# Qervas/cn_chess_ai

Hardware: AMD Instinct MI355X
Metric: env steps/sec + DQN updates/sec at 8192 parallel games, 1/2/4/8 MI355X (higher is better)
Workload: dtype f32

## Files before the change

### cn_chess_ai_amd/csrc/xq_dqn.hip

```cpp
#include "xq_internal.h"
#include <hip/hip_ext.h>
#include "xq_gemm.hip.h"
#include "xq_screen.hip.h"
#include "xq_gemm_dma.hip.h"
#include "xq_l0grad.hip.h"

#include <algorithm>
#include <cmath>
#include <mutex>
#include <random>
#include <unordered_map>

namespace xq { struct TailArgs; struct ClipRecord; }
struct xq_dqn {
    int ns = 0, nl = 0;
    int L[XQ_MAX_LAYERS + 1] = {0};
    size_t nw = 0, nb = 0;
    size_t wo[XQ_MAX_LAYERS] = {0}, bo[XQ_MAX_LAYERS] = {0};
    double lr = 1e-3, gamma = 0.99;
    uint64_t seed = 0;
    hipStream_t stream = nullptr;
    bool own_stream = false;
    hipStream_t side = nullptr;
    hipStream_t cur = nullptr;
// ... 1452 lines not shown
        g.M = d->L[ll + 1]; g.N = d->L[ll]; g.K = n;
        g.A = d->deltas[ll]; g.lda = d->L[ll + 1];
        g.B = outs[ll - 1]; g.ldb = d->L[ll];
        return grad_gemm<L_MCONTIG>(d, g, G + d->g_wh[ll], "gemm_grad_hidden", d->slabs + off_h[ll], &d->pend_hidden[ll]);
    };
    const bool defer_grad = nl == 3;
    int waiting = -1;
    for (int l = nl - 3; l >= 0; --l) {
        tail_begin(d);
        XQ_TRY(hidden_deltas(d, n, d->deltas[l + 1], d->L[l + 2], d->L[l + 2], mode, l, l));
        if (defer_grad) { if (waiting >= 0) XQ_TRY(add_grad(waiting)); waiting = l + 1; }
        else XQ_TRY(add_grad(l + 1));
        if (l == nl - 3) add_out_grad();
        if (l == 0 && l0_mfma_shape(d, n)) {
            XQ_TRY(ensure_l0_mfma(d, n));
            TailArgs& T = *d->tail;
            const int chunk0 = l0_chunk_of(n), kpad = (n + chunk0 - 1) / chunk0 * chunk0;
            T.sel_boards = d->gboards; T.sel_n = n; T.sel_kpad = kpad; T.sel_out = d->l0_sel; T.n_sel = kpad / 64;
            d->tail_bytes += (double)n * 48 + 2.0 * l0sel_elems(kpad);
            d->tail_lds = std::max(d->tail_lds, (size_t)64 * 13 * sizeof(uint32_t));
            d->l0_sel_done = true;
        }
        XQ_TRY(tail_launch(d, false, "td_tail_deltas"));
    }
    tail_begin(d);
    XQ_TRY(l0_gradient(d, n, G + d->g_w0));
    if (waiting >= 0) XQ_TRY(add_grad(waiting));
    if (nl < 3) add_out_grad();
    BiasJobs bj;
    for (int l = 0; l <= nl - 2; ++l) bj.add(d->deltas[l], d->L[l + 1], d->L[l + 1], G + d->g_bh[l]);
    d->pend_bh = xq_dqn::PendingSlab();
    XQ_TRY(bias_grads(d, bj, n, &d->pend_bh));
    return tail_launch(d, true, "td_tail_l0");
}


struct TdStep {
    const int32_t* action_to; const float* reward; const uint8_t* done; SlotSrc slots; const PerOpts* per;
    int n, mode, sel_net, nl, Hl, NO; bool dbl, bf;
    bool big_tiles;
    int n_partial;
    size_t bias_lds;
    float* outs[XQ_MAX_LAYERS]; uint16_t* outs_bf[XQ_MAX_LAYERS];
    float* touts[XQ_MAX_LAYERS]; uint16_t* touts_bf[XQ_MAX_LAYERS];
    float* t2outs[XQ_MAX_LAYERS]; uint16_t* t2outs_bf[XQ_MAX_LAYERS];
    const float* view; long long view_ld; int view_kmax;
};

static int screen_guard_tick(xq_dqn* d, int n, bool* screened) {
    XQ_TRY(ensure_screen_capacity(d, n));
    if (d->scr_guard_pending && d->scr_host_steps % kScreenCheckEvery == 0 && d->scr_host_steps != d->scr_guard_queued_at) {
        XQ_HIP(hipEventSynchronize(d->scr_guard_ev));
        d->scr_guard_pending = false;
        unsigned long long h[2];
        screen_stat_sums_of(d, d->scr_guard_host, h);
        const double ds = (double)(d->scr_guard_samples - d->scr_seen[0]);
        if (ds > 0 && ((double)(h[0] - d->scr_seen[1]) > kScreenMaxPairs * ds || (double)(h[1] - d->scr_seen[2]) > kScreenMaxWhole * ds)) {
            d->scr_hold = kScreenHoldSteps;
            d->scr_fallbacks += 1;
        }
        if (ds > 0) {
            const double share = (double)(h[1] - d->scr_seen[2]) / ds;
            if (share > 0.25) d->scr_stage_whole = true; else if (share < 0.10) d->scr_stage_whole = false;
        }
        d->scr_seen[0] = d->scr_guard_samples; d->scr_seen[1] = h[0]; d->scr_seen[2] = h[1];
    }
    *screened = d->scr_hold == 0;
    if (d->scr_hold > 0) --d->scr_hold;
    return XQ_OK;
}

static int screen_shadow_job(xq_dqn* d, int sel_net, int parity, ShadowJob* shadow) {
    const int NO = d->nout(), nl = d->nl;
    const bool full = d->scr_static_net != sel_net;
    if (full) XQ_HIP(hipMemsetAsync(d->scr_wmax + 4, 0, 2 * sizeof(unsigned), d->cur));
    memset(shadow, 0, sizeof *shadow);
    shadow->W = d->wl(sel_net, nl - 1); shadow->bias = d->bl(sel_net, nl - 1); shadow->NO = NO; shadow->K = d->hlast(); shadow->Wb = d->scr_wb;
    shadow->w_dyn = d->scr_wmax + parity; shadow->b_dyn = d->scr_wmax + 2 + parity;
    shadow->w_stat = d->scr_wmax + 4; shadow->b_stat = d->scr_wmax + 5;
    shadow->nblocks = full ? (NO + kShadowRows - 1) / kShadowRows : std::min((int)kShadowDynBlocks, (NO + kShadowRows - 1) / kShadowRows);
    d->scr_static_net = sel_net;
    return XQ_OK;
}

static int launch_screen(xq_dqn* d, const ScreenArgs& a, int mode, hipEvent_t start, hipEvent_t stop) {
    using ScreenKernel = void (*)(ScreenArgs);
    static const ScreenKernel kerns[3][2] = {{screen_top2_kernel<1, 2, SCR_TOP2>, screen_top2_kernel<2, 1, SCR_TOP2>},
                                             {screen_top2_kernel<1, 2, SCR_ARG>, screen_top2_kernel<2, 1, SCR_ARG>},
                                             {screen_top2_kernel<1, 2, SCR_MAX>, screen_top2_kernel<2, 1, SCR_MAX>}};
    const ScreenKernel kern = kerns[mode][a.K == 256 ? 0 : 1];
    XQ_TRY(ensure_max_dynamic_lds(kern, 160 * 1024));
    hipExtLaunchKernelGGL(kern, dim3(a.panels * a.ranges), dim3(512), screen_lds_bytes(a), d->cur, start, stop, 0, a);
    XQ_HIP(hipGetLastError());
    return XQ_OK;
}

static int colmax_persistent_grid(const xq_dqn* d, GemmArgs& g, int tiles_m, int total) {
    g.a_vec = g.b_vec = 1; g.k_chunk = g.K;
    g.bias_padded = ((((uintptr_t)g.bias) % 16 == 0) && (g.M % 4) == 0) ? 1 : 0;
    const int grid = std::min(total, 2 * d->ncu);
    if (grid >= 2 && (grid & 1) == 0 && total >= 4 * grid) {
        g.prio_split = grid / 2;
        g.prio_tiles = (total / 2) / tiles_m * tiles_m;
        if (g.prio_tiles <= 0 || g.prio_tiles >= total) { g.prio_split = 0; g.prio_tiles = 0; }
    }
    return grid;
}

static int qmax_screened(xq_dqn* d, const TdStep& s, bool scr_new, int parity, bool* td_fused) {
    const int n = s.n, NO = s.NO, Hl = s.Hl, nl = s.nl;
    const float *W = d->wl(s.sel_net, nl - 1), *bias = d->bl(s.sel_net, nl - 1);
    const int tiles_m = (NO + 127) / 128, total = tiles_m * ((n + 127) / 128);
    const int G = scr_new ? 2 * ((NO + 63) / 64) : 4 * tiles_m;
    long long ldp = n;
    int scr_ranges = 0, scr_gpr = 0;
    if (scr_new) {
        ScreenArgs a; memset(&a, 0, sizeof a);
        a.W = d->scr_wb; a.A = d->scr_ab; a.a_frag = 1; a.bias = bias;
        a.P1 = d->scr_p1; a.P2 = d->scr_p2; a.R = d->scr_R; a.na = d->scr_na;
        screen_geometry(NO, n, Hl, d->ncu, a);
        ldp = a.ldp = screen_padded_samples(n, Hl);
        scr_ranges = a.ranges; scr_gpr = 2 * a.cpr;
        ProfScope ps(d, "gemm_qmax_screen", 2.0 * NO * (double)n * Hl, 2.0 * ((double)NO * Hl + (double)n * Hl) + 8.0 * G * n, true);
        XQ_TRY(launch_screen(d, a, SCR_TOP2, ps.start(), ps.stop()));
    } else {
        GemmArgs g; memset(&g, 0, sizeof g);
        g.M = NO; g.N = n;
        g.K = Hl / 2; g.lda = g.ldb = Hl / 2;
        g.A = reinterpret_cast<const float*>(d->scr_wb.p); g.B = reinterpret_cast<const float*>(d->scr_ab.p);
        g.bias = bias;
        g.partial = d->scr_p1; g.partial2 = d->scr_p2;
        const int grid = colmax_persistent_grid(d, g, tiles_m, total);
        ProfScope ps(d, "gemm_qmax_screen", 2.0 * g.M * g.N * Hl, 2.0 * ((double)g.M * Hl + (double)g.N * Hl) + 8.0 * G * g.N);
        hipLaunchKernelGGL((gemm_colmax_persistent_kernel<2, 2, DT_BF16, CM_TOP2>), dim3(grid), dim3(256), s.bias_lds, d->cur, g, tiles_m, total);
        XQ_HIP(hipGetLastError());
    }
    {
        ProfScope ps(d, "qmax_refine", 2.0 * n * Hl * 3, 12.0 * G * n + 4.0 * n * Hl, true);
        const dim3 grid((n + kRefineSamples - 1) / kRefineSamples);
        const bool stage = scr_new && Hl == 256 && (int)grid.x <= d->ncu && (d->refine_stage > 0 || (d->refine_stage < 0 && d->scr_stage_whole));
        const size_t lds = refine_cand_words(G) * sizeof(uint32_t) + refine_wlist_bytes(G) + (stage ? refine_stage_bytes() : 0);
        const float* a_last = s.touts[nl - 2];
        if (scr_new) {
            TdFused T; memset(&T, 0, sizeof T);
            *td_fused = d->td_tail && Hl == 256 && !s.per && !d->bf16_bwd();
            if (*td_fused) {
                const int lt = nl - 2;
                T.src = s.slots; T.action_to = s.action_to; T.reward = s.reward; T.done = s.done;
                T.a_s = s.outs[lt]; T.w_out = d->wl(XQ_NET_ONLINE, nl - 1); T.b_out = d->bl(XQ_NET_ONLINE, nl - 1);
                T.view = s.view; T.view_ld = s.view_ld; T.view_kmax = s.view_kmax; T.gamma = (float)d->gamma;
                T.dtop = d->deltas[lt]; T.dsc = d->dsc; T.act = d->act_mb; T.qsa = d->qsa; T.yv = d->yv; T.lossv = d->lossv;
            }
            const int whole_mode = stage ? 2 : 1;
            const auto kern = *td_fused ? qmax_refine2_kernel<256, true> : Hl == 256 ? qmax_refine2_kernel<256> : qmax_refine2_kernel<512>;
            XQ_TRY(ensure_max_dynamic_lds(kern, 152 * 1024));
            hipExtLaunchKernelGGL(kern, grid, dim3(256), lds, d->cur, ps.start(), ps.stop(), 0, d->scr_R.p, scr_ranges, scr_gpr, d->scr_p1.p, d->scr_p2.p,
                                  G, n, ldp, d->scr_na.p, a_last, Hl, W, bias, NO, d->scr_wmax.p, parity, d->zmax.p, d->scr_stats.p, T, whole_mode);
        } else {
            const bool small = G <= 8 * 32;
            const auto kern = Hl == 256 ? (small ? qmax_refine_kernel<256, 32> : qmax_refine_kernel<256, 64>)
                            : Hl == 512 ? (small ? qmax_refine_kernel<512, 32> : qmax_refine_kernel<512, 64>)
                                        : (small ? qmax_refine_kernel<0, 32> : qmax_refine_kernel<0, 64>);
            hipExtLaunchKernelGGL(kern, grid, dim3(256), lds, d->cur, ps.start(), ps.stop(), 0, d->scr_p1.p, d->scr_p2.p, G, n, ldp, a_last, Hl,
                                  W, bias, NO, d->scr_wmax.p, parity, d->zmax.p, d->scr_stats.p);
        }
        XQ_HIP(hipGetLastError());
    }
    d->scr_host_steps += 1; d->scr_host_samples += (unsigned long long)n;
    if (d->scr_host_steps % kScreenCheckEvery == 0 && !d->scr_guard_pending) {
        XQ_HIP(hipMemcpyAsync(d->scr_guard_host, d->scr_stats, (size_t)2 * d->scr_stat_blocks * sizeof(unsigned long long), hipMemcpyDeviceToHost, d->cur));
        XQ_HIP(hipEventRecord(d->scr_guard_ev, d->cur));
        d->scr_guard_pending = true; d->scr_guard_samples = d->scr_host_samples; d->scr_guard_queued_at = d->scr_host_steps;
    }
    return XQ_OK;
}

static int qmax_exact(xq_dqn* d, const TdStep& s, bool bf_frag, bool gate_early) {
    const int n = s.n, NO = s.NO, Hl = s.Hl, nl = s.nl;
    const bool bf = s.bf, dbl = s.dbl;
    long long part_ld = n;
    int n_part = s.n_partial;
    if (bf && (Hl == 256 || Hl == 512) && n >= 1024) {
        ScreenArgs a; memset(&a, 0, sizeof a);
        a.W = d->wl_bf(s.sel_net, nl - 1); a.A = s.touts_bf[nl - 2]; a.a_frag = bf_frag ? 1 : 0; a.bias = d->bl(s.sel_net, nl - 1);
        a.P1 = d->partial; a.P2 = reinterpret_cast<float*>(d->partial_idx.p);
        screen_geometry(NO, n, Hl, d->ncu, a);
        part_ld = a.ldp = screen_padded_samples(n, Hl);
        n_part = 2 * a.nchunks;
        ProfScope ps(d, "gemm_qmax_rowmax", 2.0 * NO * (double)n * Hl, 2.0 * ((double)NO * Hl + (double)n * Hl) + 8.0 * n_part * n, true);
        XQ_TRY(launch_screen(d, a, dbl ? SCR_ARG : SCR_MAX, ps.start(), ps.stop()));
    } else {
        GemmArgs g; memset(&g, 0, sizeof g);
        g.M = NO; g.N = n;
        g.K = bf ? Hl / 2 : Hl; g.lda = g.ldb = g.K;
        g.A = bf ? reinterpret_cast<const float*>(d->wl_bf(s.sel_net, nl - 1)) : d->wl(s.sel_net, nl - 1);
        g.B = bf ? reinterpret_cast<const float*>(s.touts_bf[nl - 2]) : s.touts[nl - 2];
        g.bias = d->bl(s.sel_net, nl - 1);
        g.partial = d->partial;
        g.partial_idx = dbl ? d->partial_idx : nullptr;
        if (s.big_tiles && (g.K % GBK) == 0 && vec_ok(g.A, g.lda) && vec_ok(g.B, g.ldb) && s.bias_lds <= 40 * 1024) {
            const int tiles_m = (NO + 127) / 128, total = tiles_m * ((n + 127) / 128);
            const int grid = colmax_persistent_grid(d, g, tiles_m, total);
            ProfScope ps(d, "gemm_qmax_rowmax", 2.0 * g.M * g.N * Hl, (bf ? 2.0 : 4.0) * ((double)g.M * Hl + (double)g.N * Hl) + 8.0 * tiles_m * g.N);
            const auto kern = bf ? (dbl ? gemm_colmax_persistent_kernel<2, 2, DT_BF16, CM_ARG> : gemm_colmax_persistent_kernel<2, 2, DT_BF16, CM_MAX>)
                                 : (dbl ? gemm_colmax_persistent_kernel<2, 2, DT_F32, CM_ARG> : gemm_colmax_persistent_kernel<2, 2, DT_F32, CM_MAX>);
            hipLaunchKernelGGL(kern, dim3(grid), dim3(256), s.bias_lds, d->cur, g, tiles_m, total);
            XQ_HIP(hipGetLastError());
        } else if (bf) XQ_GEMM((launch_gemm<L_KCONTIG, L_KCONTIG, EPI_COLMAX, DT_BF16>(d, g, 1, "gemm_qmax_rowmax")));
        else XQ_GEMM((launch_gemm<L_KCONTIG, L_KCONTIG, EPI_COLMAX>(d, g, 1, "gemm_qmax_rowmax")));
    }
    if (!d->late_gate && !gate_early) XQ_HIP(hipEventRecord(d->ev_qmax, d->stream));
    {
        ProfScope ps(d, "colmax_reduce", (double)n * n_part, (dbl ? 8.0 : 4.0) * n * (n_part + kReduceParts));
        hipLaunchKernelGGL(colmax_reduce_kernel, dim3((n + 63) / 64, kReduceParts), dim3(256), 0, d->cur, d->partial,
                           dbl ? d->partial_idx : nullptr, n_part, n, part_ld, d->zmax, d->zidx);
        XQ_HIP(hipGetLastError());
    }
    return XQ_OK;
}

static int td_delta(xq_dqn* d, const TdStep& s, int zparts) {
    const int n = s.n, nl = s.nl, Hl = s.Hl;
    const int lt = nl - 2;
    ProfScope ps(d, "td_target_delta", 4.0 * n * Hl, (double)n * (Hl * 16 + s.n_partial * 4));
    TdExtra X; memset(&X, 0, sizeof X);
    X.nout = s.NO;
    if (s.dbl) {
        X.double_dqn = 1; X.partial_idx = d->zidx;
        X.bout_t = d->bl(XQ_NET_TARGET, nl - 1);
        if (s.bf) { X.wout_t_bf = d->wl_bf(XQ_NET_TARGET, nl - 1); X.alast_t_bf = s.t2outs_bf[lt]; }
        else { X.wout_t = d->wl(XQ_NET_TARGET, nl - 1); X.alast_t = s.t2outs[lt]; }
    }
    if (s.bf) X.wout_bf = d->wl_bf(XQ_NET_ONLINE, nl - 1);
    if (d->bf16_bwd()) X.dtop_bf = d->deltas_bf[lt];
    if (const PerOpts* per = s.per) {
        X.is_w = per->is_w; X.is_wmax = per->is_wmax; X.prio = per->prio; X.pmax_live = per->pmax_live;
        X.per_eps = per->eps; X.per_alpha = per->alpha;
    }
    hipLaunchKernelGGL(td_delta_kernel, dim3((n + 3) / 4), dim3(256), 0, d->cur, n, s.slots, s.action_to, s.reward, s.done,
                       s.outs[lt], Hl, d->wl(XQ_NET_ONLINE, nl - 1), d->bl(XQ_NET_ONLINE, nl - 1), d->zmax, zparts,
                       (float)d->gamma, s.view, s.view_ld, s.view_kmax, d->deltas[lt], d->dsc, d->act_mb, d->qsa, d->yv, d->lossv, X);
    XQ_HIP(hipGetLastError());
    return XQ_OK;
}

static int td_gradients_fork(xq_dqn* d, const TdStep& s) {
    const int n = s.n, nl = s.nl;
    float* G = d->grads_td;
    XQ_HIP(hipEventRecord(d->ev_fork, d->stream));
    XQ_HIP(hipStreamWaitEvent(d->side, d->ev_fork, 0));
    if (nl >= 3) XQ_TRY(hidden_deltas(d, n, d->deltas[nl - 2], d->L[nl - 1], d->L[nl - 1], s.mode, nl - 3));
    XQ_HIP(hipEventRecord(d->ev_delta, d->stream));
    const size_t n0 = (size_t)d->L[0] * d->L[1];
    if (!d->comm) XQ_TRY(l0_gradient(d, n, G + d->g_w0));
    d->cur = d->side;
    const int rc = side_gradients(d, n, s.outs, G);
    d->cur = d->stream;
    if (rc != XQ_OK) return rc;
    if (d->comm) XQ_TRY(comm_allreduce_on(d->comm, G + n0, d->n_grads_td - n0, d->side));
    XQ_HIP(hipEventRecord(d->ev_join, d->side));
    if (d->comm) {
        XQ_TRY(l0_gradient(d, n, G + d->g_w0));
        XQ_TRY(comm_allreduce_on(d->comm, G, n0, d->stream));
    }
    XQ_HIP(hipStreamWaitEvent(d->stream, d->ev_join, 0));
    return XQ_OK;
}

static int td_grads_impl(xq_dqn* d, const uint32_t* boards, const uint32_t* next_boards, const int32_t* action_to,
                         const float* reward, const uint8_t* done, SlotSrc slots, int n, int td_net, int mode, const PerOpts* per) {
    if (!d || !boards || !next_boards || !action_to || !reward || !done || n <= 0)
        return fail(XQ_ERR_INVALID_ARGUMENT, "xq_dqn_td_grads: bad argument");
    if (td_net != XQ_TD_ONLINE_NET && td_net != XQ_TD_TARGET_NET && td_net != XQ_TD_DOUBLE) return fail(XQ_ERR_INVALID_ARGUMENT, "bad td_net");
    if (mode != XQ_BACKPROP_REFERENCE && mode != XQ_BACKPROP_TEXTBOOK) return fail(XQ_ERR_INVALID_ARGUMENT, "bad backprop mode");
    if (d->nout() < 96) return fail(XQ_ERR_INVALID_ARGUMENT, "TD path needs >= 96 outputs (action.to indexes outputs 0..89)");
    if (mode == XQ_BACKPROP_REFERENCE) XQ_TRY(check_reference_topology(d));
    const bool dbl = td_net == XQ_TD_DOUBLE, bf = d->bf16();
    d->l0_split_done = d->l0_sel_done = false;
    d->late_gate = d->comm != nullptr && tail_eligible(d, n) &&
                   (d->exchange_overlap == 1 ||
                    (d->exchange_overlap < 0 && (d->exch_calibrated ? d->exch_late : comm_world(d->comm) > 1)));
    XQ_TRY(ensure_capacity(d, n));
    XQ_TRY(ensure_ext_capacity(d, n, dbl));
    const int nl = d->nl, Hl = d->hlast(), NO = d->nout();
    if (bf && (Hl & 1)) return fail(XQ_ERR_INVALID_ARGUMENT, "bf16 Q-net needs even layer widths");
    TdStep s;
    s.action_to = action_to; s.reward = reward; s.done = done; s.slots = slots; s.per = per;
    s.n = n; s.mode = mode; s.nl = nl; s.Hl = Hl; s.NO = NO; s.dbl = dbl; s.bf = bf; s.sel_net = td_net == XQ_TD_TARGET_NET ? XQ_NET_TARGET : XQ_NET_ONLINE;
    for (int l = 0; l + 1 < nl; ++l) {
        s.outs[l] = d->acts[l]; s.outs_bf[l] = d->acts_bf[l];
        s.touts[l] = bf ? nullptr : d->tacts[l & 1]; s.touts_bf[l] = d->tacts_bf[l & 1];
        s.t2outs[l] = bf ? nullptr : d->t2acts[l & 1]; s.t2outs_bf[l] = d->t2acts_bf[l & 1];
    }
    s.big_tiles = (long long)((NO + 127) / 128) * ((n + 127) / 128) >= 512;
    s.n_partial = 2 * (s.big_tiles ? (NO + 127) / 128 : (NO + 63) / 64);
    s.bias_lds = (size_t)((NO + 127) / 128) * 128 * sizeof(float);
    s.view = d->wrest(XQ_NET_ONLINE) + (d->wo[nl - 1] - d->wo[1]);
    s.view_ld = mode == XQ_BACKPROP_REFERENCE ? d->L[nl - 2] : d->L[nl - 1]; s.view_kmax = mode == XQ_BACKPROP_REFERENCE ? d->L[nl - 1] : NO;
    const bool want_screen = d->qmax_mode == XQ_QMAX_SCREENED && !bf && !dbl && s.big_tiles && (Hl % 64) == 0 && Hl <= 1024 &&
                             s.bias_lds <= 40 * 1024 && (NO + 127) / 128 * 4 <= 8 * kRefineMaxPerThread;
    bool screened = false;
    if (want_screen) XQ_TRY(screen_guard_tick(d, n, &screened));
    const int parity = (int)(d->scr_host_steps & 1);
    const bool scr_new = screened && (Hl == 256 || Hl == 512);
    ShadowJob shadow;
    if (screened) XQ_TRY(screen_shadow_job(d, s.sel_net, parity, &shadow));
    const bool bf_frag = bf && nl >= 3 && (Hl == 256 || Hl == 512) && n >= 1024 && (n % kBgBM) == 0 && (d->L[nl - 2] % kBgBK) == 0;
// ... 413 lines not shown
```

### cn_chess_ai_amd/csrc/xq_refine.hip.h

```cpp
#pragma once

namespace xq {

constexpr float kScreenEps = 0.0078125f * 1.0625f;
constexpr float kScreenBiasEps = 0.001953125f;
enum { kScreenCheckEvery = 32, kScreenHoldSteps = 512 };
constexpr double kScreenMaxPairs = 24.0, kScreenMaxWhole = 1.0;

__device__ __forceinline__ int float_order_key(float f) {
    const int b = __builtin_bit_cast(int, f);
    return b ^ ((b >> 31) & 0x7fffffff);
}
__device__ __forceinline__ float float_from_key(int k) { return __builtin_bit_cast(float, k ^ ((k >> 31) & 0x7fffffff)); }
__device__ __forceinline__ float wave_sum_f32(float v) {
#pragma unroll
    for (int off = 32; off >= 1; off >>= 1) v += __shfl_xor(v, off, 64);
    return v;
}

enum { kRefineSamples = 32, kRefineMaxPerThread = 64 };

template <int KFIX>
__device__ __forceinline__ float quarter_dot(const float* __restrict__ ap, const float* __restrict__ wp, int K, int ql) {
    float acc = 0.f;
    if (KFIX > 0) {
        constexpr int NT = KFIX > 0 ? KFIX / 64 : 1;
        float4 x[NT], w[NT];
#pragma unroll
        for (int t = 0; t < KFIX / 64; ++t) {
            x[t] = *reinterpret_cast<const float4*>(ap + t * 64 + ql * 4);
            w[t] = *reinterpret_cast<const float4*>(wp + t * 64 + ql * 4);
        }
#pragma unroll
        for (int t = 0; t < KFIX / 64; ++t) {
            acc = fmaf(x[t].x, w[t].x, acc); acc = fmaf(x[t].y, w[t].y, acc);
            acc = fmaf(x[t].z, w[t].z, acc); acc = fmaf(x[t].w, w[t].w, acc);
        }
    } else {
        for (int k = ql * 4; k < K; k += 64) {
            const float4 x = *reinterpret_cast<const float4*>(ap + k);
            const float4 w = *reinterpret_cast<const float4*>(wp + k);
            acc = fmaf(x.x, w.x, acc); acc = fmaf(x.y, w.y, acc); acc = fmaf(x.z, w.z, acc); acc = fmaf(x.w, w.w, acc);
        }
    }
    return acc;
}
__device__ __forceinline__ float quarter_sum(float v) {
#pragma unroll
    for (int off = 8; off >= 1; off >>= 1) v += __shfl_xor(v, off, 64);
    return v;
}
__device__ __forceinline__ int screen_row(int g, int code) {
    const int q = code & 15;
    return (g >> 2) * 128 + ((g >> 1) & 1) * 64 + 4 * (g & 1) + (code >> 4) * 32 + (q & 3) + 8 * (q >> 2);
}

template <int KFIX, int NPT>
__global__ __launch_bounds__(256) void qmax_refine_kernel(const float* __restrict__ P1, const float* __restrict__ P2, int G, int n, long long ldp,
                                                          const float* __restrict__ a_last, int K, const float* __restrict__ W,
                                                          const float* __restrict__ bias, int NO, unsigned* __restrict__ wm, int parity,
                                                          float* __restrict__ zmax, unsigned long long* __restrict__ stats) {
    extern __shared__ __attribute__((aligned(16))) uint32_t cand[];
    uint16_t* wlist = reinterpret_cast<uint16_t*>(cand + (size_t)G * kRefineSamples);
    __shared__ float sv[8][32];
    __shared__ float na[32], thr[32];
    __shared__ int best[32];
    __shared__ int cnt, nexp;
    const int tid = (int)threadIdx.x;
    const int sl = tid & 31, phase = tid >> 5;
    const int ql = tid & 15, quarter = tid >> 4;
    const int b0 = (int)blockIdx.x * kRefineSamples;
    const int b = b0 + sl;
    const bool ok = b < n;
    if (tid == 0) { cnt = 0; nexp = 0; if (blockIdx.x == 0) { wm[parity ^ 1] = 0u; wm[2 + (parity ^ 1)] = 0u; } }
    unsigned long long st_pairs = 0, st_whole = 0;
    if (tid == 0) { st_pairs = stats[2 * blockIdx.x]; st_whole = stats[2 * blockIdx.x + 1]; }
    if (tid < 32) best[tid] = (int)0x80000000;
    float v[NPT], v2[NPT];
    const int bc = min(b, n - 1);
#pragma unroll
    for (int u = 0; u < NPT; ++u) {
        const int g = min(phase + 8 * u, G - 1);
        v[u] = P1[(long long)g * ldp + bc];
        v2[u] = P2[(long long)g * ldp + bc];
    }
#pragma unroll
    for (int u = 0; u < NPT; ++u)
        if (!ok || phase + 8 * u >= G) { v[u] = kColmaxPadBias; v2[u] = kColmaxPadBias; }
#pragma unroll
    for (int r = 0; r < 2; ++r) {
        const int i = quarter + 16 * r;
        const float* ap = a_last + (long long)min(b0 + i, n - 1) * K;
        const float ss = quarter_sum(quarter_dot<KFIX>(ap, ap, K, ql));
        if (ql == 0) na[i] = ss;
    }
    float m = kColmaxPadBias;
#pragma unroll
    for (int u = 0; u < NPT; ++u) m = fmaxf(m, v[u]);
    sv[phase][sl] = m;
    __syncthreads();
    if (tid < 32) {
        m = sv[0][sl];
#pragma unroll
        for (int p = 1; p < 8; ++p) m = fmaxf(m, sv[p][sl]);
        const float wmx = fmaxf(__builtin_bit_cast(float, wm[parity]), __builtin_bit_cast(float, wm[4]));
        const float bmx = fmaxf(__builtin_bit_cast(float, wm[2 + parity]), __builtin_bit_cast(float, wm[5]));
        const float B = kScreenEps * sqrtf(na[sl]) * wmx + kScreenBiasEps * bmx;
        float t0 = m - 2.f * B * 1.03125f - 1.52587890625e-05f * (fabsf(m) + 2.f * B);
        if (!(t0 == t0)) t0 = -__builtin_inff();
        thr[sl] = b0 + sl < n ? t0 : __builtin_inff();
    }
    __syncthreads();
    {
        const float t = thr[sl];
#pragma unroll
        for (int u = 0; u < NPT; ++u) {
            const int g = phase + 8 * u;
            if (v[u] >= t) {
                if (v2[u] >= t) wlist[atomicAdd(&nexp, 1)] = (uint16_t)(sl | (g << 5));
                else cand[atomicAdd(&cnt, 1)] = (uint32_t)sl | ((uint32_t)screen_row(g, (int)(__builtin_bit_cast(uint32_t, v[u]) & 31u)) << 5);
            }
        }
    }
    __syncthreads();
    const int singles = cnt, wholes = nexp;
    for (int e0 = 0; e0 < singles; e0 += 64) {
        float z[4];
        int s2[4], row[4];
        bool live[4];
#pragma unroll
        for (int r = 0; r < 4; ++r) {
            const int e = e0 + quarter + 16 * r;
            live[r] = e < singles;
            const uint32_t ent = cand[live[r] ? e : 0];
            s2[r] = (int)(ent & 31u);
            row[r] = min((int)(ent >> 5), NO - 1);
            z[r] = quarter_dot<KFIX>(a_last + (long long)(b0 + s2[r]) * K, W + (long long)row[r] * K, K, ql);
        }
#pragma unroll
        for (int r = 0; r < 4; ++r) {
            z[r] = quarter_sum(z[r]) + bias[row[r]];
            if (live[r] && ql == 0 && z[r] == z[r]) atomicMax(&best[s2[r]], float_order_key(z[r]));
        }
    }
    for (int e = 0; e < wholes; ++e) {
        const int ent = wlist[e];
        const int s2 = ent & 31, g = ent >> 5;
        float zb = kColmaxPadBias;
#pragma unroll
        for (int r = 0; r < 2; ++r) {
            const int row = screen_row(g, quarter + 16 * r);
            const int rc = min(row, NO - 1);
            const float z = quarter_sum(quarter_dot<KFIX>(a_last + (long long)(b0 + s2) * K, W + (long long)rc * K, K, ql)) + bias[rc];
            if (row < NO) zb = fmaxf(zb, z);
        }
        if (ql == 0) atomicMax(&best[s2], float_order_key(zb));
    }
    __syncthreads();
    if (tid < 32 && ok) zmax[b] = float_from_key(best[sl]);
    if (tid == 0) {
        stats[2 * blockIdx.x] = st_pairs + (unsigned long long)(singles + wholes);
        stats[2 * blockIdx.x + 1] = st_whole + (unsigned long long)wholes;
    }
}

struct TdFused {
    SlotSrc src;
    const int32_t* action_to; const float* reward; const uint8_t* done;
    const float* a_s;
    const float* w_out; const float* b_out;
    const float* view; long long view_ld; int view_kmax;
    float gamma;
    float* dtop; float* dsc; int32_t* act; float* qsa; float* yv; float* lossv;
};
__host__ __device__ inline size_t refine_cand_words(int G) { const size_t w = (size_t)G * 32; return w < 8192 ? 8192 : w; }
__host__ __device__ inline size_t refine_wlist_bytes(int G) { return ((size_t)G * 32 * sizeof(uint16_t) + 15) & ~(size_t)15; }
__host__ __device__ inline size_t refine_stage_bytes() { return (size_t)3 * 32 * 256 * sizeof(float); }
template <int KFIX, bool TD = false>
__global__ __launch_bounds__(256) void qmax_refine2_kernel(const float* __restrict__ R, int ranges, int gpr ,
                                                           const float* __restrict__ P1, const float* __restrict__ P2, int G, int n, long long ldp,
                                                           const float* __restrict__ na_all, const float* __restrict__ a_last, int K,
                                                           const float* __restrict__ W, const float* __restrict__ bias, int NO,
                                                           unsigned* __restrict__ wm, int parity, float* __restrict__ zmax,
                                                           unsigned long long* __restrict__ stats, const TdFused T, int whole_mode) {
    extern __shared__ __attribute__((aligned(16))) uint32_t cand[];
    uint16_t* wlist = reinterpret_cast<uint16_t*>(cand + refine_cand_words(G));
    __shared__ float sv[8][32];
    __shared__ float thr[32];
    __shared__ int best[32];
    __shared__ int cnt, nexp;
    __shared__ unsigned gbits[256];
    __shared__ unsigned long long gpop[4];
    const int tid = (int)threadIdx.x;
    const int sl = tid & 31, phase = tid >> 5;
    const int ql = tid & 15, quarter = tid >> 4;
    const int b0 = (int)blockIdx.x * kRefineSamples;
    const int b = b0 + sl;
    const bool ok = b < n;
    const int bc = min(b, n - 1);
    if (tid == 0) { cnt = 0; nexp = 0; if (blockIdx.x == 0) { wm[parity ^ 1] = 0u; wm[2 + (parity ^ 1)] = 0u; } }
    unsigned long long st_pairs = 0, st_whole = 0;
    if (tid == 0) { st_pairs = stats[2 * blockIdx.x]; st_whole = stats[2 * blockIdx.x + 1]; }
    if (tid < 32) best[tid] = (int)0x80000000;
    const bool stage_ok = KFIX > 0 && G <= 256;
    gbits[tid] = 0u;
    const int td_lane = tid & 63, td_w = tid >> 6;
    int td_a = -1; float td_r = 0.f, td_bo = 0.f; bool td_dn = false;
    float zq[8];
    if (TD) {
        static_assert(!TD || KFIX == 256, "fused TD delta: 256-wide last hidden layer");
        if (td_lane < 8) {
            const int bb = min(b0 + td_w * 8 + td_lane, n - 1);
            const int sslot = slot_of(T.src, bb);
            td_a = T.action_to[sslot];
            td_r = T.reward[sslot];
            td_dn = T.done[sslot] != 0;
            td_bo = T.b_out[(td_a >= 0 && td_a < 96) ? td_a : 0];
        }
#pragma unroll
        for (int i = 0; i < 8; ++i) {
            const int bb = min(b0 + td_w * 8 + i, n - 1);
            const int a = __shfl(td_a, i, 64);
            const int ac = (a >= 0 && a < 96) ? a : 0;
            const float4 av = *reinterpret_cast<const float4*>(T.a_s + (long long)bb * 256 + td_lane * 4);
            const float4 wv = *reinterpret_cast<const float4*>(T.w_out + (long long)ac * 256 + td_lane * 4);
            zq[i] = (av.x * wv.x + av.y * wv.y) + (av.z * wv.z + av.w * wv.w);
        }
    }
    float m = kColmaxPadBias;
    for (int r = phase; r < ranges; r += 8) m = fmaxf(m, R[(long long)r * ldp + bc]);
    sv[phase][sl] = m;
    __syncthreads();
    if (tid < 32) {
        m = sv[0][sl];
#pragma unroll
        for (int p = 1; p < 8; ++p) m = fmaxf(m, sv[p][sl]);
        const float wmx = fmaxf(__builtin_bit_cast(float, wm[parity]), __builtin_bit_cast(float, wm[4]));
        const float bmx = fmaxf(__builtin_bit_cast(float, wm[2 + parity]), __builtin_bit_cast(float, wm[5]));
        const float B = kScreenEps * sqrtf(na_all[bc]) * wmx + kScreenBiasEps * bmx;
        float t0 = m - 2.f * B * 1.03125f - 1.52587890625e-05f * (fabsf(m) + 2.f * B);
        if (!(t0 == t0)) t0 = -__builtin_inff();
        thr[sl] = ok ? t0 : __builtin_inff();
    }
    __syncthreads();
    {
        const float t = thr[sl];
        for (int r = phase; r < ranges; r += 8) {
            if (R[(long long)r * ldp + bc] < t) continue;
            const int g0 = r * gpr, g1 = min(G, g0 + gpr);
            for (int g = g0; g < g1; g += 16) {
                float v[16], v2[16];
#pragma unroll
                for (int u = 0; u < 16; ++u) v[u] = P1[(long long)min(g + u, g1 - 1) * ldp + bc];
#pragma unroll
                for (int u = 0; u < 16; ++u) v2[u] = (g + u < g1 && v[u] >= t) ? P2[(long long)(g + u) * ldp + bc] : 0.f;
#pragma unroll
                for (int u = 0; u < 16; ++u) {
                    if (g + u < g1 && v[u] >= t) {
                        if (v2[u] >= t) { wlist[atomicAdd(&nexp, 1)] = (uint16_t)(sl | ((g + u) << 5)); if (stage_ok) atomicOr(&gbits[g + u], 1u << sl); }
                        else cand[atomicAdd(&cnt, 1)] = (uint32_t)sl | ((uint32_t)screen_row(g + u, (int)(__builtin_bit_cast(uint32_t, v[u]) & 31u)) << 5);
                    }
                }
            }
        }
    }
    __syncthreads();
    const int singles = cnt, wholes = nexp;
    for (int e0 = 0; e0 < singles; e0 += 64) {
        float z[4];
        int s2[4], row[4];
        bool live[4];
#pragma unroll
        for (int r = 0; r < 4; ++r) {
            const int e = e0 + quarter + 16 * r;
            live[r] = e < singles;
            const uint32_t ent = cand[live[r] ? e : 0];
            s2[r] = (int)(ent & 31u);
            row[r] = min((int)(ent >> 5), NO - 1);
            z[r] = quarter_dot<KFIX>(a_last + (long long)(b0 + s2[r]) * K, W + (long long)row[r] * K, K, ql);
        }
#pragma unroll
        for (int r = 0; r < 4; ++r) {
            z[r] = quarter_sum(z[r]) + bias[row[r]];
            if (live[r] && ql == 0 && z[r] == z[r]) atomicMax(&best[s2[r]], float_order_key(z[r]));
        }
    }
    const bool staged_pass = stage_ok && KFIX == 256 && wholes >= 8 && whole_mode == 2;
    if (staged_pass) {
        float* Wt0 = reinterpret_cast<float*>(cand);
        float* At = reinterpret_cast<float*>(reinterpret_cast<unsigned char*>(wlist) + refine_wlist_bytes(G));
        {
            const unsigned long long m = __ballot(__popc(gbits[tid]) >= 8);
            if ((tid & 63) == 0) gpop[tid >> 6] = m;
        }
        __syncthreads();
        unsigned long long gm[4] = {gpop[0], gpop[1], gpop[2], gpop[3]};
        bool a_staged = false;
        for (;;) {
            int gs[3];
#pragma unroll
            for (int u = 0; u < 3; ++u) {
                gs[u] = -1;
#pragma unroll
                for (int wv = 0; wv < 4; ++wv)
                    if (gs[u] < 0 && gm[wv]) { gs[u] = wv * 64 + __builtin_ctzll(gm[wv]); gm[wv] &= gm[wv] - 1; }
            }
            if (gs[0] < 0) break;
            float bj[3][2];
#pragma unroll
            for (int u = 0; u < 3; ++u)
#pragma unroll
                for (int r = 0; r < 2; ++r) bj[u][r] = gs[u] >= 0 ? bias[min(screen_row(gs[u], quarter + 16 * r), NO - 1)] : 0.f;
#pragma unroll
            for (int half = 0; half < 2; ++half) {
                float4 ra[4], rw0[4], rw1[4], rw2[4];
#pragma unroll
                for (int q = 0; q < 4; ++q) {
                    const int i = (half * 4 + q) * 256 + tid, j = i >> 6, c = i & 63;
                    ra[q] = *reinterpret_cast<const float4*>(a_last + (long long)min(b0 + j, n - 1) * K + 4 * c);
                    rw0[q] = *reinterpret_cast<const float4*>(W + (long long)min(screen_row(gs[0], j), NO - 1) * K + 4 * c);
                    rw1[q] = *reinterpret_cast<const float4*>(W + (long long)min(screen_row(gs[1] >= 0 ? gs[1] : gs[0], j), NO - 1) * K + 4 * c);
                    rw2[q] = *reinterpret_cast<const float4*>(W + (long long)min(screen_row(gs[2] >= 0 ? gs[2] : gs[0], j), NO - 1) * K + 4 * c);
                }
#pragma unroll
                for (int q = 0; q < 4; ++q) {
                    const int i = (half * 4 + q) * 256 + tid;
                    if (!a_staged) reinterpret_cast<float4*>(At)[i] = ra[q];
                    if (gs[0] >= 0) reinterpret_cast<float4*>(Wt0)[i] = rw0[q];
                    if (gs[1] >= 0) reinterpret_cast<float4*>(At + 1 * 32 * 256)[i] = rw1[q];
                    if (gs[2] >= 0) reinterpret_cast<float4*>(At + 2 * 32 * 256)[i] = rw2[q];
                }
            }
            a_staged = true;
            __syncthreads();
#pragma unroll
            for (int u = 0; u < 3; ++u) {
                if (gs[u] < 0) continue;
                const float* Wt = u == 0 ? Wt0 : At + u * 32 * 256;
                unsigned left = gbits[gs[u]];
                while (left) {
                    const int s2 = __builtin_ctz(left);
                    left &= left - 1;
                    float zb = kColmaxPadBias;
#pragma unroll
                    for (int r = 0; r < 2; ++r) {
                        const int j = quarter + 16 * r;
                        const float z = quarter_sum(quarter_dot<KFIX>(At + s2 * 256, Wt + j * 256, K, ql)) + bj[u][r];
                        if (screen_row(gs[u], j) < NO) zb = fmaxf(zb, z);
                    }
                    if (ql == 0) atomicMax(&best[s2], float_order_key(zb));
                }
            }
            __syncthreads();
        }
    }
    for (int e = 0; e < wholes; ++e) {
        const int ent = wlist[e];
        const int s2 = ent & 31, g = ent >> 5;
        if (staged_pass && __popc(gbits[g]) >= 8) continue;
        float zb = kColmaxPadBias;
#pragma unroll
        for (int r = 0; r < 2; ++r) {
            const int row = screen_row(g, quarter + 16 * r);
            const int rc = min(row, NO - 1);
            const float z = quarter_sum(quarter_dot<KFIX>(a_last + (long long)(b0 + s2) * K, W + (long long)rc * K, K, ql)) + bias[rc];
            if (row < NO) zb = fmaxf(zb, z);
        }
        if (ql == 0) atomicMax(&best[s2], float_order_key(zb));
    }
    __syncthreads();
    if (tid < 32 && ok) zmax[b] = float_from_key(best[sl]);
    if (tid == 0) {
        stats[2 * blockIdx.x] = st_pairs + (unsigned long long)(singles + wholes);
        stats[2 * blockIdx.x + 1] = st_whole + (unsigned long long)wholes;
    }
    if (TD) {
        float4 av[8], vv[8];
#pragma unroll
        for (int i = 0; i < 8; ++i) {
            const int bb = min(b0 + td_w * 8 + i, n - 1);
            const int a = __shfl(td_a, i, 64);
            const bool has_view = a >= 0 && a < 96 && a < T.view_kmax;
            av[i] = *reinterpret_cast<const float4*>(T.a_s + (long long)bb * 256 + td_lane * 4);
            vv[i] = has_view ? *reinterpret_cast<const float4*>(T.view + (long long)a * T.view_ld + td_lane * 4) : make_float4(0.f, 0.f, 0.f, 0.f);
        }
#pragma unroll
        for (int i = 0; i < 8; ++i) {
            const int bb = b0 + td_w * 8 + i;
            const int a = __shfl(td_a, i, 64);
            const float r = __shfl(td_r, i, 64), bo = __shfl(td_bo, i, 64);
            const bool dn = __shfl((int)td_dn, i, 64) != 0;
            const bool live = a >= 0 && a < 96;
            float z = zq[i];
#pragma unroll
            for (int off = 32; off > 0; off >>= 1) z += __shfl_xor(z, off, 64);
            const float zm = float_from_key(best[td_w * 8 + i]);
            float q = 0.f, y = 0.f, delta = 0.f;
            if (live) {
                q = tanhf(z + bo);
                y = dn ? r : r + T.gamma * tanhf(zm);
                delta = (q - y) * (1.f - q * q) * 1.f;
            }
            if (bb < n) {
                float4 o = make_float4(0.f, 0.f, 0.f, 0.f);
                if (live && a < T.view_kmax) {
                    o.x = delta * vv[i].x * (1.f - av[i].x * av[i].x); o.y = delta * vv[i].y * (1.f - av[i].y * av[i].y);
                    o.z = delta * vv[i].z * (1.f - av[i].z * av[i].z); o.w = delta * vv[i].w * (1.f - av[i].w * av[i].w);
                }
                *reinterpret_cast<float4*>(T.dtop + (long long)bb * 256 + td_lane * 4) = o;
                if (td_lane == 0) {
                    T.dsc[bb] = delta;
                    T.act[bb] = live ? a : -1;
                    T.qsa[bb] = q; T.yv[bb] = y;
                    T.lossv[bb] = live ? 0.5f * (q - y) * (q - y) : 0.f;
                }
            }
        }
    }
}


}
```

Baseline: 46.62 million.

## Cut register pressure in refine kernel via STAGE template and early TD reduction

Adds a STAGE template parameter so the LDS staging path is only compiled into variants that use it, letting non-staged variants use fewer registers. The TD z-reduction moves earlier so only one float per lane (td_z) stays live instead of eight zq values. The singles loop processes two rows per quarter instead of four, and an asm barrier keeps lane indices from being rematerialised. Together these aim to lower VGPR usage and raise occupancy, at the cost of more loop iterations and extra kernel instantiations.

```diff
diff --git a/cn_chess_ai_amd/csrc/xq_dqn.hip b/cn_chess_ai_amd/csrc/xq_dqn.hip
--- a/cn_chess_ai_amd/csrc/xq_dqn.hip
+++ b/cn_chess_ai_amd/csrc/xq_dqn.hip
@@ -1628,7 +1628,8 @@
                 T.dtop = d->deltas[lt]; T.dsc = d->dsc; T.act = d->act_mb; T.qsa = d->qsa; T.yv = d->yv; T.lossv = d->lossv;
             }
             const int whole_mode = stage ? 2 : 1;
-            const auto kern = *td_fused ? qmax_refine2_kernel<256, true> : Hl == 256 ? qmax_refine2_kernel<256> : qmax_refine2_kernel<512>;
+            const auto kern = *td_fused ? (stage ? qmax_refine2_kernel<256, true, true> : qmax_refine2_kernel<256, true>)
+                            : Hl == 256 ? (stage ? qmax_refine2_kernel<256, false, true> : qmax_refine2_kernel<256>) : qmax_refine2_kernel<512>;
             XQ_TRY(ensure_max_dynamic_lds(kern, 152 * 1024));
             hipExtLaunchKernelGGL(kern, grid, dim3(256), lds, d->cur, ps.start(), ps.stop(), 0, d->scr_R.p, scr_ranges, scr_gpr, d->scr_p1.p, d->scr_p2.p,
                                   G, n, ldp, d->scr_na.p, a_last, Hl, W, bias, NO, d->scr_wmax.p, parity, d->zmax.p, d->scr_stats.p, T, whole_mode);
diff --git a/cn_chess_ai_amd/csrc/xq_refine.hip.h b/cn_chess_ai_amd/csrc/xq_refine.hip.h
--- a/cn_chess_ai_amd/csrc/xq_refine.hip.h
+++ b/cn_chess_ai_amd/csrc/xq_refine.hip.h
@@ -176,7 +176,7 @@
 __host__ __device__ inline size_t refine_cand_words(int G) { const size_t w = (size_t)G * 32; return w < 8192 ? 8192 : w; }
 __host__ __device__ inline size_t refine_wlist_bytes(int G) { return ((size_t)G * 32 * sizeof(uint16_t) + 15) & ~(size_t)15; }
 __host__ __device__ inline size_t refine_stage_bytes() { return (size_t)3 * 32 * 256 * sizeof(float); }
-template <int KFIX, bool TD = false>
+template <int KFIX, bool TD = false, bool STAGE = false>
 __global__ __launch_bounds__(256) void qmax_refine2_kernel(const float* __restrict__ R, int ranges, int gpr ,
                                                            const float* __restrict__ P1, const float* __restrict__ P2, int G, int n, long long ldp,
                                                            const float* __restrict__ na_all, const float* __restrict__ a_last, int K,
@@ -202,11 +202,11 @@
     unsigned long long st_pairs = 0, st_whole = 0;
     if (tid == 0) { st_pairs = stats[2 * blockIdx.x]; st_whole = stats[2 * blockIdx.x + 1]; }
     if (tid < 32) best[tid] = (int)0x80000000;
-    const bool stage_ok = KFIX > 0 && G <= 256;
+    const bool stage_ok = STAGE && KFIX > 0 && G <= 256;
     gbits[tid] = 0u;
     const int td_lane = tid & 63, td_w = tid >> 6;
     int td_a = -1; float td_r = 0.f, td_bo = 0.f; bool td_dn = false;
-    float zq[8];
+    float zq[8], td_z = 0.f;
     if (TD) {
         static_assert(!TD || KFIX == 256, "fused TD delta: 256-wide last hidden layer");
         if (td_lane < 8) {
@@ -230,6 +230,15 @@
     float m = kColmaxPadBias;
     for (int r = phase; r < ranges; r += 8) m = fmaxf(m, R[(long long)r * ldp + bc]);
     sv[phase][sl] = m;
+    if (TD) {
+#pragma unroll
+        for (int i = 0; i < 8; ++i) {
+            float z = zq[i];
+#pragma unroll
+            for (int off = 32; off > 0; off >>= 1) z += __shfl_xor(z, off, 64);
+            if (td_lane == i) td_z = z;
+        }
+    }
     __syncthreads();
     if (tid < 32) {
         m = sv[0][sl];
@@ -266,12 +275,12 @@
     }
     __syncthreads();
     const int singles = cnt, wholes = nexp;
-    for (int e0 = 0; e0 < singles; e0 += 64) {
-        float z[4];
-        int s2[4], row[4];
-        bool live[4];
-#pragma unroll
-        for (int r = 0; r < 4; ++r) {
+    for (int e0 = 0; e0 < singles; e0 += 32) {
+        float z[2];
+        int s2[2], row[2];
+        bool live[2];
+#pragma unroll
+        for (int r = 0; r < 2; ++r) {
             const int e = e0 + quarter + 16 * r;
             live[r] = e < singles;
             const uint32_t ent = cand[live[r] ? e : 0];
@@ -280,7 +289,7 @@
             z[r] = quarter_dot<KFIX>(a_last + (long long)(b0 + s2[r]) * K, W + (long long)row[r] * K, K, ql);
         }
 #pragma unroll
-        for (int r = 0; r < 4; ++r) {
+        for (int r = 0; r < 2; ++r) {
             z[r] = quarter_sum(z[r]) + bias[row[r]];
             if (live[r] && ql == 0 && z[r] == z[r]) atomicMax(&best[s2[r]], float_order_key(z[r]));
         }
@@ -376,25 +385,25 @@
     }
     if (TD) {
         float4 av[8], vv[8];
+        int td_lane2 = td_lane, td_w2 = td_w;
+        asm volatile("" : "+v"(td_a), "+v"(td_lane2), "+v"(td_w2));
 #pragma unroll
         for (int i = 0; i < 8; ++i) {
-            const int bb = min(b0 + td_w * 8 + i, n - 1);
+            const int bb = min(b0 + td_w2 * 8 + i, n - 1);
             const int a = __shfl(td_a, i, 64);
             const bool has_view = a >= 0 && a < 96 && a < T.view_kmax;
-            av[i] = *reinterpret_cast<const float4*>(T.a_s + (long long)bb * 256 + td_lane * 4);
-            vv[i] = has_view ? *reinterpret_cast<const float4*>(T.view + (long long)a * T.view_ld + td_lane * 4) : make_float4(0.f, 0.f, 0.f, 0.f);
+            av[i] = *reinterpret_cast<const float4*>(T.a_s + (long long)bb * 256 + td_lane2 * 4);
+            vv[i] = has_view ? *reinterpret_cast<const float4*>(T.view + (long long)a * T.view_ld + td_lane2 * 4) : make_float4(0.f, 0.f, 0.f, 0.f);
         }
 #pragma unroll
         for (int i = 0; i < 8; ++i) {
-            const int bb = b0 + td_w * 8 + i;
+            const int bb = b0 + td_w2 * 8 + i;
             const int a = __shfl(td_a, i, 64);
             const float r = __shfl(td_r, i, 64), bo = __shfl(td_bo, i, 64);
             const bool dn = __shfl((int)td_dn, i, 64) != 0;
             const bool live = a >= 0 && a < 96;
-            float z = zq[i];
-#pragma unroll
-            for (int off = 32; off > 0; off >>= 1) z += __shfl_xor(z, off, 64);
-            const float zm = float_from_key(best[td_w * 8 + i]);
+            const float z = __shfl(td_z, i, 64);
+            const float zm = float_from_key(best[td_w2 * 8 + i]);
             float q = 0.f, y = 0.f, delta = 0.f;
             if (live) {
                 q = tanhf(z + bo);
@@ -407,8 +416,8 @@
                     o.x = delta * vv[i].x * (1.f - av[i].x * av[i].x); o.y = delta * vv[i].y * (1.f - av[i].y * av[i].y);
                     o.z = delta * vv[i].z * (1.f - av[i].z * av[i].z); o.w = delta * vv[i].w * (1.f - av[i].w * av[i].w);
                 }
-                *reinterpret_cast<float4*>(T.dtop + (long long)bb * 256 + td_lane * 4) = o;
-                if (td_lane == 0) {
+                *reinterpret_cast<float4*>(T.dtop + (long long)bb * 256 + td_lane2 * 4) = o;
+                if (td_lane2 == 0) {
                     T.dsc[bb] = delta;
                     T.act[bb] = live ? a : -1;
                     T.qsa[bb] = q; T.yv[bb] = y;
```

After: 47.00 million, median of 6. About the same (+0.8%).
